# qingpingmo/OCN

Measured on AMD Instinct MI355X. Metric: candidate-edges/sec (CN predictor fwd), ogbl-collab shape, higher is better.
Workload: dtype f32

## Files before the change

### include/ocn_hip.h

```cpp
#ifndef OCN_HIP_H
#define OCN_HIP_H

#include <stdint.h>

#ifdef __cplusplus
extern "C" {
#endif

#define OCN_ABI_VERSION 9
#define OCN_EINVAL (-1)
#define OCN_ECAP   (-2)

#define OCN_ST_CAP  1
#define OCN_ST_SCAN 2
#define OCN_SCAN_POISON (-1)

#define OCN_F_CN1 1u
#define OCN_F_CN2 2u

int ocn_abi_version(void);

int64_t ocn_scan_workspace_bytes(int64_t n);

int ocn_zero_regions(void* const* ptrs, const int64_t* bytes, int32_t n, void* stream);
// ... 135 lines not shown
int64_t ocn_two_hop_window_cols(void);
int ocn_two_hop_diff_count(const int64_t* rowptrA, const int32_t* colA, const int64_t* rowptrM, const int32_t* colM,
                           int64_t n_cols, const int64_t* rows, int64_t Q, int32_t drop_self,
                           int64_t window_cols , int32_t* count , void* stream);
int ocn_two_hop_diff_fill(const int64_t* rowptrA, const int32_t* colA, const int64_t* rowptrM, const int32_t* colM,
                          int64_t n_cols, const int64_t* rows, int64_t Q, int32_t drop_self,
                          int64_t window_cols , const int64_t* off ,
                          int64_t* edges , void* stream);
int64_t ocn_two_hop_sums_window_cols(void);
int ocn_two_hop_sums_fill(const int64_t* rowptrA, const int32_t* colA, const int64_t* rowptrM, const int32_t* colM,
                          int64_t n_cols, const int64_t* rows, int64_t Q, int32_t drop_self,
                          int64_t window_cols ,
                          const float* w ,
                          int32_t wcol , const int64_t* off ,
                          int64_t* edges , float* val , void* stream);
int64_t ocn_frontier_window_cols(void);
int ocn_frontier_count(const int64_t* rowptrA, const int32_t* colA, const int64_t* rowptrM, const int32_t* colM, int64_t n_cols,
                       const int64_t* rows, int64_t Q, int32_t drop_self, int64_t window_cols ,
                       const int64_t* ptrF , const int64_t* nodeF ,
                       const int64_t* ptrS , const int64_t* nodeS ,
                       int32_t* count , void* stream);
int ocn_frontier_sums_fill(const int64_t* rowptrA, const int32_t* colA, const int64_t* rowptrM, const int32_t* colM,
                           int64_t n_cols, const int64_t* rows, int64_t Q, int32_t drop_self,
                           int64_t window_cols , const int64_t* ptrF ,
                           const int64_t* nodeF , const float* valF ,
                           const int64_t* ptrS , const int64_t* nodeS ,
                           const float* valS , const int64_t* off ,
                           int64_t* edges , float* val , void* stream);
int32_t ocn_segment_topk_max_k(void);
int ocn_segment_topk(const float* scores, const int64_t* ptr, int64_t Q, int32_t k, float* top_val, int64_t* top_pos,
                     void* stream);
int ocn_segment_rank(const float* scores, const int64_t* ptr, const int64_t* edges , int64_t Q,
                     const int64_t* tptr , const int64_t* tnode , int64_t P,
                     int64_t* rank , int64_t* pos , void* stream);

int ocn_philox4x32(const uint32_t* ctr , uint32_t key0, uint32_t key1, int64_t n, uint32_t* out ,
                   void* stream);
int ocn_complement_count(const int64_t* rowptrK, const int32_t* colK, int64_t n_cols, int32_t* count ,
                         void* stream);
int32_t ocn_sample_stage_cols(void);
int ocn_sample_complement_rows(const int64_t* rowptrK, const int32_t* colK, int64_t n_cols, const int64_t* rows, int64_t Q,
                               int64_t per, int64_t q0, uint64_t seed, int64_t* out , void* stream);
int ocn_sample_complement_pairs(const int64_t* rowptrK, const int32_t* colK, int64_t n_cols,
                                const int64_t* cptr , int64_t T, int64_t t0, uint64_t seed,
                                int64_t* out , void* stream);

int64_t ocn_sample_two_hop_window_cols(void);
int ocn_sample_two_hop(const int64_t* rowptrA, const int32_t* colA, const int64_t* rowptrM, const int32_t* colM, int64_t n_cols,
                       const int64_t* rows, int64_t Q, int32_t drop_self, int64_t window_cols ,
                       const int64_t* sptr , const int64_t* sid , int64_t q0, uint64_t seed,
                       int32_t* count , int64_t* out , void* stream);

int ocn_gather_schedule(const int32_t* gcost, int64_t n_groups, int64_t segment, int32_t* perm, void* stream);

int ocn_cn_weights_cn6(uint64_t* histA, uint64_t* histB, int64_t N, const float* innerprod, int32_t* scalars,
                       float* nip_out, const float* s2_exact , const float* s3_exact ,
                       void* stream);
int ocn_cn_gather3(const int64_t* rowptrA, const int32_t* colA, const int64_t* src, const int64_t* dst,
                   const int64_t* order, int64_t B, const int64_t* off, const uint8_t* flagsA,
                   const uint8_t* flagsB, const float* weightsA, const float* weightsB, const float* nip,
                   const float* h, int32_t H, float* xcn1, float* xcn2, float* xcn3, float* xij, void* stream);

int ocn_cn3_flags(const int64_t* rowptrA, const int32_t* colA, const int64_t* rowptrT, const int32_t* colT,
                  const uint32_t* bitmapP, int64_t bm_stride_words, const int64_t* src, const int64_t* dst,
                  const int64_t* order , int64_t B, int64_t n_cols, const int64_t* off, uint8_t* flags,
                  int64_t flags_cap, uint64_t* hist , int32_t* cnt3, int32_t* status,
                  const int64_t* nds , const int64_t* chunk_off , void* stream);

int ocn_cn_gather3_backward(const int64_t* rowptrA, const int32_t* colA, const int64_t* src, const int64_t* dst,
                            const int64_t* order, int64_t B, const int64_t* off, const uint8_t* flagsA,
                            const uint8_t* flagsB, const float* weightsA, const float* weightsB, const float* nip,
                            const float* h, int32_t H, const float* g1, const float* g2, const float* g3,
                            const float* g4, float* dh, void* stream);

int ocn_cn_gather_backward(const int64_t* rowptrA, const int32_t* colA,
                           const int64_t* src, const int64_t* dst, const int64_t* order, int64_t B,
                           const int64_t* off, const uint8_t* flags, const int32_t* wc,
                           const float* weights, const float* h, int32_t H,
                           const float* g1, const float* g2, const float* g3, float* dh, void* stream);

int64_t ocn_cn_gather_backward_det_workspace_bytes(int64_t N, int64_t B, int64_t flags_cap);
int ocn_cn_gather_backward_det(const int64_t* rowptrA, const int32_t* colA, const int64_t* src, const int64_t* dst,
                               int64_t B, const int64_t* off, const uint8_t* flags, const int32_t* wc, int64_t flags_cap,
                               const float* weights, const float* h, int64_t N, int32_t H, const float* g1,
                               const float* g2, const float* g3, float* dh, void* workspace, void* stream);
int64_t ocn_cn_gather_backward_det_keys_offset(int64_t N);
int ocn_cn_gather_backward_det_lists(const int64_t* rowptrA, const int32_t* colA, const int64_t* src, const int64_t* dst,
                                     int64_t B, const int64_t* off, const uint8_t* flags, int64_t flags_cap, int64_t N,
                                     void* workspace, void* stream);

int ocn_spmm_csr(const int64_t* rowptr, const int32_t* col, const float* val, int64_t n_rows,
                 const float* x, int32_t F, const float* pre, const float* post,
                 int32_t mode, int32_t edge_scale, int32_t self_mode,
                 float* y, void* stream);

int ocn_spmm_csr_rows(const int64_t* rowptr, const int32_t* col, const float* val, int64_t n_rows,
                      const float* x, int32_t F, const float* pre, const float* post,
                      int32_t mode, int32_t edge_scale, int32_t self_mode,
                      const int64_t* rows, int64_t n_list, float* y, void* stream);

int ocn_spmm_csr_max_arg(const int64_t* rowptr, const int32_t* col, const float* val, int64_t n_rows,
                         const float* x, int32_t F, float* y, int32_t* arg, void* stream);
int ocn_spmm_max_backward(const int64_t* rowptrT, const int32_t* colT, const float* valT, int64_t n_rows,
                          const int32_t* arg, const float* g, int32_t F, float* gx, void* stream);

int ocn_sddmm_csr(const int64_t* rowptr, const int32_t* col, const float* val , int64_t n_rows,
// ... 143 lines not shown
```

### ocn_amd/_lib.py

```python
from __future__ import annotations

import ctypes
import glob
import os
import subprocess
from ctypes import c_float, c_int32, c_int64, c_void_p

_HERE = os.path.dirname(os.path.abspath(__file__))
_ROOT = os.path.dirname(_HERE)
LIB_PATH = os.environ.get("OCN_LIB_PATH", os.path.join(_HERE, "libocn_hip.so"))
CSRC = os.path.join(_HERE, "csrc")
INCLUDE = os.path.join(_ROOT, "include")

_P = c_void_p
ABI_VERSION = 9
SIGNATURES = {
    "ocn_abi_version": (c_int32, []),
    "ocn_scan_workspace_bytes": (c_int64, [c_int64]),
    "ocn_zero_regions": (c_int32, [_P, _P, c_int32, _P]),
    "ocn_check_edges": (c_int32, [_P, _P, c_int64, c_int64, c_int64, _P, _P]),
    "ocn_edge_offsets": (c_int32, [_P, _P, c_int64, _P, _P, _P]),
    "ocn_class_order": (c_int32, [_P, _P, _P, c_int64, _P, _P, _P, _P, _P, _P]),
    "ocn_scan_i32": (c_int32, [_P, c_int64, _P, _P, _P]),
    "ocn_order_workspace_bytes": (c_int64, [c_int64]),
# ... 4 lines not shown
    "ocn_cn_flags": (c_int32, [_P, _P, _P, _P, _P, _P, _P, c_int64, _P, c_int64, _P, _P, _P, c_int64, c_int64, _P, _P, c_int64, _P,
                               _P, _P, _P, _P, _P, _P]),
    "ocn_cn_flags_rec": (c_int32, [_P, _P, _P, _P, _P, _P, _P, c_int64, _P, c_int64, _P, _P, _P, c_int64, c_int64, _P, _P, c_int64, _P,
                                   _P, _P, _P, _P, _P, _P]),
    "ocn_chunk_offsets": (c_int32, [_P, _P, _P, _P, c_int64, _P, _P, _P]),
    "ocn_walk_chunk": (c_int32, []),
    "ocn_cn_walk_flags": (c_int32, [_P, _P, _P, _P, _P, _P, c_int64, _P, _P, _P, c_int64, _P, _P, c_int64, _P, _P, _P,
                                    _P, _P]),
    "ocn_neighbor_degree_sum": (c_int32, [_P, _P, c_int64, _P, _P]),
    "ocn_walk_prep_max_batch": (c_int32, []),
    "ocn_cn_flags_small_graph_cols": (c_int32, []),
    "ocn_cn_flags_pair_min_batch": (c_int64, [c_int64]),
    "ocn_walk_prep": (c_int32, [_P, _P, _P, _P, c_int64, c_int32, _P, _P, _P, _P, _P, _P, _P, _P, _P, _P, _P, _P, _P]),
    "ocn_cn_walk_group": (c_int32, [_P, _P, _P, _P, _P, c_int64, _P, _P, _P, _P, _P, _P, _P, c_int64, _P, _P, _P, _P]),
    "ocn_walk_rev_offsets": (c_int32, [_P, _P, _P, _P, _P, c_int64, _P, _P, _P]),
    "ocn_cn_weights_cn5": (c_int32, [_P, c_int64, _P, _P, c_int32, _P, _P]),
    "ocn_cn5_column_stats": (c_int32, [_P, c_int64, _P, _P]),
    "ocn_cn_colsum_workspace_bytes": (c_int64, [c_int64, c_int64]),
    "ocn_cn_colsum_exact": (c_int32, [_P, _P, _P, c_int64, _P, _P, _P, _P, c_int64, _P, c_int64, _P, _P, _P, _P, _P, _P, _P]),
    "ocn_cn_weights_cn7": (c_int32, [_P, c_int64, c_float, _P, _P, _P]),
    "ocn_cn_gather": (c_int32, [_P, _P, _P, _P, _P, c_int64, _P, _P, _P, _P, _P, c_int32, c_int64, _P, _P, _P, _P, _P,
                                _P, _P, _P, _P, _P]),
    "ocn_cn8_pool": (c_int32, [_P, _P, _P, _P, _P, _P, _P, c_int64, _P, c_int64, _P, _P, _P, c_int64, c_int64, _P, c_int32, _P, _P,
                               _P, _P, _P, _P]),
    "ocn_cn_pool_frozen": (c_int32, [_P, _P, _P, _P, _P, _P, _P, c_int64, _P, c_int64, _P, _P, _P, c_int64, c_int64, _P, _P, c_int32, _P,
                                     _P, _P, _P, _P, _P]),
    "ocn_cn_attribution": (c_int32, [_P, _P, _P, _P, c_int64, _P, _P, _P, c_int64, _P, _P, c_int32, _P, _P, _P, _P, _P]),
    "ocn_cn_node_sums": (c_int32, [_P, _P, _P, _P, _P, _P, _P, c_int64, _P, c_int64, _P, _P, _P, c_int64, c_int64, _P, _P, _P, _P, _P,
                                   _P, _P]),
    "ocn_row_diff_stage_cols": (c_int32, []),
    "ocn_row_diff_count": (c_int32, [_P, _P, _P, _P, _P, c_int64, c_int32, _P, _P]),
    "ocn_row_diff_fill": (c_int32, [_P, _P, _P, _P, _P, c_int64, c_int32, _P, _P, _P]),
    "ocn_two_hop_window_cols": (c_int64, []),
    "ocn_two_hop_diff_count": (c_int32, [_P, _P, _P, _P, c_int64, _P, c_int64, c_int32, c_int64, _P, _P]),
    "ocn_two_hop_diff_fill": (c_int32, [_P, _P, _P, _P, c_int64, _P, c_int64, c_int32, c_int64, _P, _P, _P]),
    "ocn_two_hop_sums_window_cols": (c_int64, []),
    "ocn_two_hop_sums_fill": (c_int32, [_P, _P, _P, _P, c_int64, _P, c_int64, c_int32, c_int64, _P, c_int32, _P, _P, _P, _P]),
    "ocn_frontier_window_cols": (c_int64, []),
    "ocn_frontier_count": (c_int32, [_P, _P, _P, _P, c_int64, _P, c_int64, c_int32, c_int64, _P, _P, _P, _P, _P, _P]),
    "ocn_frontier_sums_fill": (c_int32, [_P, _P, _P, _P, c_int64, _P, c_int64, c_int32, c_int64, _P, _P, _P, _P, _P, _P, _P, _P, _P,
                                         _P]),
    "ocn_segment_topk_max_k": (c_int32, []),
    "ocn_segment_topk": (c_int32, [_P, _P, c_int64, c_int32, _P, _P, _P]),
    "ocn_segment_rank": (c_int32, [_P, _P, _P, c_int64, _P, _P, c_int64, _P, _P, _P]),
    "ocn_philox4x32": (c_int32, [_P, ctypes.c_uint32, ctypes.c_uint32, c_int64, _P, _P]),
    "ocn_complement_count": (c_int32, [_P, _P, c_int64, _P, _P]),
    "ocn_sample_stage_cols": (c_int32, []),
    "ocn_sample_complement_rows": (c_int32, [_P, _P, c_int64, _P, c_int64, c_int64, c_int64, ctypes.c_uint64, _P, _P]),
    "ocn_sample_complement_pairs": (c_int32, [_P, _P, c_int64, _P, c_int64, c_int64, ctypes.c_uint64, _P, _P]),
    "ocn_sample_two_hop_window_cols": (c_int64, []),
    "ocn_sample_two_hop": (c_int32, [_P, _P, _P, _P, c_int64, _P, c_int64, c_int32, c_int64, _P, _P, c_int64, ctypes.c_uint64, _P, _P,
                                     _P]),
    "ocn_gather_schedule": (c_int32, [_P, c_int64, c_int64, _P, _P]),
    "ocn_coo_to_csr_workspace_bytes": (c_int64, [c_int64, c_int64, c_int32, c_int32]),
    "ocn_coo_to_csr": (c_int32, [_P, _P, c_int64, c_int64, c_int64, c_int32, c_int32, _P, _P, _P, _P, _P]),
    "ocn_wgrad_workspace_bytes": (c_int64, [c_int64, c_int32, c_int32]),
    "ocn_wgrad": (c_int32, [_P, c_int64, _P, c_int64, c_int64, c_int32, c_int32, _P, _P, _P, _P]),
    "ocn_cn_weights_cn6": (c_int32, [_P, _P, c_int64, _P, _P, _P, _P, _P, _P]),
    "ocn_cn_gather3": (c_int32, [_P, _P, _P, _P, _P, c_int64, _P, _P, _P, _P, _P, _P, _P, c_int32, _P, _P, _P, _P, _P]),
    "ocn_cn3_flags": (c_int32, [_P, _P, _P, _P, _P, c_int64, _P, _P, _P, c_int64, c_int64, _P, _P, c_int64, _P, _P, _P, _P, _P, _P]),
    "ocn_cn_gather3_backward": (c_int32, [_P, _P, _P, _P, _P, c_int64, _P, _P, _P, _P, _P, _P, _P, c_int32, _P, _P, _P, _P, _P, _P]),
    "ocn_cn_gather_backward": (c_int32, [_P, _P, _P, _P, _P, c_int64, _P, _P, _P, _P, _P, c_int32, _P, _P, _P, _P, _P]),
    "ocn_cn_gather_backward_det_workspace_bytes": (c_int64, [c_int64, c_int64, c_int64]),
    "ocn_cn_gather_backward_det": (c_int32, [_P, _P, _P, _P, c_int64, _P, _P, _P, c_int64, _P, _P, c_int64, c_int32, _P, _P, _P, _P,
                                             _P, _P]),
    "ocn_cn_gather_backward_det_keys_offset": (c_int64, [c_int64]),
    "ocn_cn_gather_backward_det_lists": (c_int32, [_P, _P, _P, _P, c_int64, _P, _P, c_int64, c_int64, _P, _P]),
    "ocn_ln_drop_relu_workspace_bytes": (c_int64, [c_int32]),
    "ocn_ln_drop_relu_forward": (c_int32, [_P, _P, _P, c_float, c_float, ctypes.c_uint64, c_int32, c_int64, c_int32, _P, _P, _P]),
    "ocn_ln_drop_relu_backward": (c_int32, [_P, _P, _P, _P, _P, c_float, ctypes.c_uint64, c_int32, c_int64, c_int32, _P, _P, _P, _P, _P]),
    "ocn_dropout_keep_mask": (c_int32, [ctypes.c_uint64, c_float, c_int64, _P, _P]),
    "ocn_mix3_workspace_bytes": (c_int64, []),
    "ocn_mix3_backward": (c_int32, [_P, _P, _P, _P, _P, c_int64, _P, _P, _P, _P, _P, _P]),
    "ocn_spmm_csr": (c_int32, [_P, _P, _P, c_int64, _P, c_int32, _P, _P, c_int32, c_int32, c_int32, _P, _P]),
    "ocn_spmm_csr_rows": (c_int32, [_P, _P, _P, c_int64, _P, c_int32, _P, _P, c_int32, c_int32, c_int32, _P, c_int64, _P, _P]),
    "ocn_spmm_csr_max_arg": (c_int32, [_P, _P, _P, c_int64, _P, c_int32, _P, _P, _P]),
    "ocn_spmm_max_backward": (c_int32, [_P, _P, _P, c_int64, _P, _P, c_int32, _P, _P]),
    "ocn_sddmm_csr": (c_int32, [_P, _P, _P, c_int64, _P, _P, c_int32, _P, _P, c_int32, c_int32, c_int32, _P, _P]),
    "ocn_deg_rsqrt": (c_int32, [_P, _P, c_int64, c_float, _P, _P]),
    "ocn_spgemm_max_cols": (c_int64, []),
    "ocn_spgemm_pattern_count": (c_int32, [_P, _P, c_int64, _P, _P, c_int64, _P, _P, c_int64, _P]),
    "ocn_spgemm_pattern_fill": (c_int32, [_P, _P, c_int64, _P, _P, c_int64, _P, _P, _P]),
    "ocn_spgemm_bit_rows": (c_int32, [_P, _P, c_int64, _P, _P, c_int64, _P, c_int64, _P, _P, c_int64, _P]),
    "ocn_dense_from_csr": (c_int32, [_P, _P, c_int64, c_int64, _P, _P, _P]),
    "ocn_dense_block_mm_bits": (c_int32, [_P, _P, c_int64, c_int64, c_int32, c_int32, c_int32, c_int32, c_int32, _P, c_int64, _P]),
    "ocn_bitrows_from_csr": (c_int32, [_P, _P, c_int64, _P, c_int64, _P]),
    "ocn_bitrows_count": (c_int32, [_P, c_int64, c_int64, c_int64, _P, _P]),
    "ocn_bitrows_fill": (c_int32, [_P, c_int64, c_int64, c_int64, _P, _P, _P]),
    "ocn_csr_union_count": (c_int32, [_P, _P, _P, _P, c_int64, _P, _P]),
    "ocn_csr_union_fill": (c_int32, [_P, _P, _P, _P, c_int64, _P, _P, _P]),
    "ocn_bitrows_insert_workspace_bytes": (c_int64, [c_int64]),
    "ocn_bitrows_insert": (c_int32, [_P, _P, _P, _P, _P, _P, c_int64, c_int64, _P, c_int64, _P, _P, _P]),
    "ocn_csr_minus_count": (c_int32, [_P, _P, _P, _P, c_int64, _P, _P]),
    "ocn_csr_minus_fill": (c_int32, [_P, _P, _P, _P, c_int64, _P, _P, _P]),
    "ocn_bitrows_remove_workspace_bytes": (c_int64, [c_int64]),
    "ocn_bitrows_remove": (c_int32, [_P, _P, _P, _P, _P, _P, _P, _P, _P, _P, c_int64, c_int64, _P, c_int64, _P, _P, _P]),
    "ocn_rows_neighbourhood_workspace_bytes": (c_int64, [c_int64]),
    "ocn_rows_neighbourhood": (c_int32, [_P, _P, c_int64, _P, c_int64, _P, _P, _P]),
    "ocn_bitlist_count": (c_int32, [_P, c_int64, _P, _P]),
    "ocn_bitlist_fill": (c_int32, [_P, c_int64, _P, _P, _P]),
    "ocn_rows_ln_relu": (c_int32, [_P, _P, _P, c_float, c_int32, c_int64, c_int32, _P, _P]),
    "ocn_fill_rows": (c_int32, [_P, c_int64, c_int32, _P, _P, c_int64, _P]),
    "ocn_combine3": (c_int32, [_P, _P, _P, _P, c_int64, _P, _P]),
    "ocn_linear_panel_bytes": (c_int64, [c_int32, c_int32]),
    "ocn_linear_split_weight": (c_int32, [_P, c_int32, c_int32, _P, _P]),
    "ocn_linear_bf16x6": (c_int32, [_P, c_int64, c_int32, _P, c_int32, _P, _P, _P, c_float, c_int32, _P, _P,
# ... 114 lines not shown
```

### ocn_amd/csrc/cn_pool.hip

```cpp
#include "common.h"


constexpr int GATHER_UNR = 4;
template <int LPE, int NV, int UNR = (LPE >= 64 ? 2 * GATHER_UNR : GATHER_UNR)>
__device__ __forceinline__ void pool_range(i64 p_begin, i64 p_end, i64 a0, i64 base, int gl, int gbase,
                                           const int32_t* __restrict__ colA, const uint8_t* __restrict__ flags,
                                           const int32_t* __restrict__ wc, const float4* __restrict__ weights,
                                           const float4* __restrict__ h4, i64 rowq, float4 (&acc1)[NV],
                                           float4 (&acc2)[NV], bool full2 = false) {
  constexpr int PT = (OCN_WAVE / LPE) < 8 ? (OCN_WAVE / LPE) : 8;
  f32x2 acc[NV][4];
#pragma unroll
  for (int v = 0; v < NV; ++v) {
    acc[v][0] = f32x2{acc1[v].x, acc2[v].x}; acc[v][1] = f32x2{acc1[v].y, acc2[v].y};
    acc[v][2] = f32x2{acc1[v].z, acc2[v].z}; acc[v][3] = f32x2{acc1[v].w, acc2[v].w};
  }
  for (i64 p0 = p_begin; p0 < p_end; p0 += LPE * PT) {
    int32_t k[PT];
    unsigned f[PT];
    int32_t cv[PT];
#pragma unroll
    for (int t = 0; t < PT; ++t) {
      const i64 p = p0 + t * LPE + gl;
      k[t] = 0; f[t] = 0; cv[t] = 1;
      if (p < p_end) {
        k[t] = colA[a0 + p]; f[t] = flags[base + p];
        if (wc) cv[t] = wc[base + p];
      }
      if (full2) f[t] &= ~OCN_F_CN2;
    }
    float wa[PT], wb[PT];
#pragma unroll
    for (int t = 0; t < PT; ++t) {
      wa[t] = wb[t] = 0.f;
      if (f[t]) entry_weights(f[t], weights[k[t]], (float)cv[t], wa[t], wb[t]);
    }
#pragma unroll
    for (int t = 0; t < PT; ++t) {
      const bool need = (wa[t] != 0.f) | (wb[t] != 0.f);
      unsigned long long m = __ballot(need);
      if (LPE < 64) m = (m >> gbase) & ((1ull << (LPE & 63)) - 1ull);
      while (m) {
        int bsel[UNR];
#pragma unroll
        for (int u = 0; u < UNR; ++u) {
          bsel[u] = m ? (__ffsll((long long)m) - 1) : -1;
          m &= m - 1;
        }
        int32_t kk[UNR];
        float wwa[UNR], wwb[UNR];
        float4 x[UNR][NV];
#pragma unroll
        for (int u = 0; u < UNR; ++u) {
          const int sl = gbase + (bsel[u] < 0 ? 0 : bsel[u]);
          kk[u] = __shfl(k[t], sl, OCN_WAVE);
          wwa[u] = __shfl(wa[t], sl, OCN_WAVE);
          wwb[u] = __shfl(wb[t], sl, OCN_WAVE);
          if (bsel[u] >= 0) {
            const float4* row = h4 + (i64)kk[u] * rowq + gl;
#pragma unroll
            for (int v = 0; v < NV; ++v) x[u][v] = row[v * LPE];
          }
        }
#pragma unroll
        for (int u = 0; u < UNR; ++u) {
          if (bsel[u] >= 0) {
            const f32x2 w = {wwa[u], wwb[u]};
#pragma unroll
            for (int v = 0; v < NV; ++v) {
              axpy_pair(acc[v][0], w, x[u][v].x);
              axpy_pair(acc[v][1], w, x[u][v].y);
              axpy_pair(acc[v][2], w, x[u][v].z);
              axpy_pair(acc[v][3], w, x[u][v].w);
            }
          }
        }
      }
    }
  }
#pragma unroll
  for (int v = 0; v < NV; ++v) {
    acc1[v] = make_float4(acc[v][0].x, acc[v][1].x, acc[v][2].x, acc[v][3].x);
    acc2[v] = make_float4(acc[v][0].y, acc[v][1].y, acc[v][2].y, acc[v][3].y);
  }
}

template <int LPE, int NV>
__device__ __forceinline__ void pool_store(i64 e, i64 i, i64 j, int gl, const float4* __restrict__ h4, i64 rowq,
                                           const float4 (&acc1)[NV], const float4 (&acc2)[NV],
                                           float* __restrict__ xcn1, float* __restrict__ xcn2,
                                           float* __restrict__ xij, bool st1 = true, bool st2 = true) {
  const float4* hi = h4 + i * rowq + gl;
  const float4* hj = h4 + j * rowq + gl;
  float4* o1 = reinterpret_cast<float4*>(xcn1) + e * rowq + gl;
  float4* o2 = reinterpret_cast<float4*>(xcn2) + e * rowq + gl;
  float4* o3 = reinterpret_cast<float4*>(xij) + e * rowq + gl;
#pragma unroll
  for (int v = 0; v < NV; ++v) {
    const float4 a = hi[v * LPE], b = hj[v * LPE];
    if (st1) o1[v * LPE] = acc1[v];
    if (st2) o2[v * LPE] = acc2[v];
    o3[v * LPE] = make_float4(__fmul_rn(a.x, b.x), __fmul_rn(a.y, b.y), __fmul_rn(a.z, b.z),
                              __fmul_rn(a.w, b.w));
  }
}

#define LONG_ROW 1024

template <int LPE, int NV>
__global__ __launch_bounds__(OCN_BLOCK) void cn_gather_kernel(
    const i64* __restrict__ rowptrA, const int32_t* __restrict__ colA,
    const i64* __restrict__ src, const i64* __restrict__ dst, const i64* __restrict__ order, i64 B,
    const i64* __restrict__ off, const uint8_t* __restrict__ flags, const int32_t* __restrict__ wc,
    const float4* __restrict__ weights, const float* __restrict__ h, int H,
    float* __restrict__ xcn1, float* __restrict__ xcn2, float* __restrict__ xij,
    const i64* __restrict__ out_row,
    const int32_t* __restrict__ cnt1, const int32_t* __restrict__ cnt2,
    const u64* __restrict__ rec,
    const int32_t* __restrict__ perm,
    const float* __restrict__ rowsum) {
  constexpr int GPW = OCN_WAVE / LPE;
  const int lane = threadIdx.x & 63;
  const int gl = lane % LPE;
  const int gbase = lane - gl;
  i64 bid = blockIdx.x;
  if ((gridDim.x & 7) == 0) {
    bid = (bid & 7) * (gridDim.x >> 3) + (bid >> 3);
    if (perm) bid = perm[bid];
  }
  const i64 slot = (bid * OCN_WPB + (threadIdx.x >> 6)) * GPW + lane / LPE;
  if (slot >= B) return;
  i64 e, i, j, a0, da, base;
  bool has1, has2, full2;
  if (rec) {
    const ulonglong2* rp = reinterpret_cast<const ulonglong2*>(rec + 4 * slot);
    const ulonglong2 ra = rp[0], rb = rp[1];
    e = (i64)ra.x; i = (i64)(ra.y & 0xffffffffull); j = (i64)(ra.y >> 32);
    a0 = (i64)(rb.x & ((1ull << REC_LEN_SHIFT) - 1)); da = (i64)(rb.x >> REC_LEN_SHIFT);
    base = (i64)(rb.y & ((1ull << REC_FULL2_BIT) - 1)); has1 = (rb.y >> 62) & 1ull; has2 = rb.y >> 63;
    full2 = rowsum && ((rb.y >> REC_FULL2_BIT) & 1ull);
  } else {
    e = order ? order[slot] : slot;
    i = src[e]; j = dst[e];
    a0 = rowptrA[i]; da = rowptrA[i + 1] - a0;
    base = off[e];
    has1 = !cnt1 || cnt1[e] > 0; has2 = !cnt2 || cnt2[e] > 0;
    full2 = rowsum && cnt2 && da > 0 && (i64)cnt2[e] == da;
  }
  if (da > LONG_ROW && !full2) return;
  const float4* h4 = reinterpret_cast<const float4*>(h);
  const i64 rowq = H >> 2;
  float4 acc1[NV], acc2[NV];
#pragma unroll
  for (int v = 0; v < NV; ++v) acc1[v] = acc2[v] = make_float4(0.f, 0.f, 0.f, 0.f);
  if (has1 | (has2 & !full2)) pool_range<LPE, NV>(0, da, a0, base, gl, gbase, colA, flags, wc, weights, h4, rowq, acc1, acc2, full2);
  if (full2) {
    const float4* rs = reinterpret_cast<const float4*>(rowsum) + i * rowq + gl;
#pragma unroll
    for (int v = 0; v < NV; ++v) acc2[v] = rs[v * LPE];
  }
  pool_store<LPE, NV>(out_row ? out_row[e] : e, i, j, gl, h4, rowq, acc1, acc2, xcn1, xcn2, xij,
                      !out_row || has1, !out_row || has1 || has2);
}

template <int FPL, int HF>
__device__ __forceinline__ void chain_rows(const float2* __restrict__ w, const float* __restrict__ xs, int nr,
                                           float (&acc1)[FPL], float (&acc2)[FPL]) {
  constexpr int BLK = FPL >= 4 ? 2 : 8 / FPL;
  f32x2 acc[FPL];
#pragma unroll
  for (int q = 0; q < FPL; ++q) acc[q] = f32x2{acc1[q], acc2[q]};
  auto load = [&](int r, float2 (&w8)[BLK], float (&x8)[BLK][FPL]) {
#pragma unroll
    for (int u = 0; u < BLK; ++u) {
      w8[u] = w[r + u];
#pragma unroll
      for (int q = 0; q < FPL; ++q) x8[u][q] = xs[(r + u) * HF + q];
    }
  };
  auto add = [&](const float2 (&w8)[BLK], const float (&x8)[BLK][FPL]) {
#pragma unroll
    for (int u = 0; u < BLK; ++u)
#pragma unroll
      for (int q = 0; q < FPL; ++q) axpy_pair_lds(acc[q], f32x2{w8[u].x, w8[u].y}, x8[u][q]);
  };
  const int nb = nr / BLK;
  if (nb > 0) {
    float2 wa[BLK], wb[BLK];
    float xa[BLK][FPL], xb[BLK][FPL];
    load(0, wa, xa);
    int b = 0;
    for (; b + 2 <= nb; b += 2) {
      load((b + 1) * BLK, wb, xb);
      add(wa, xa);
      if (b + 2 < nb) load((b + 2) * BLK, wa, xa);
      add(wb, xb);
    }
    if (b < nb) add(wa, xa);
  }
  for (int r = nb * BLK; r < nr; ++r) {
    const float2 wr = w[r];
#pragma unroll
    for (int q = 0; q < FPL; ++q) axpy_pair_lds(acc[q], f32x2{wr.x, wr.y}, xs[r * HF + q]);
  }
#pragma unroll
  for (int q = 0; q < FPL; ++q) { acc1[q] = acc[q].x; acc2[q] = acc[q].y; }
}

template <int LPE, int NV, bool LONG>
constexpr int gather_wave_wpb() { return LONG ? 1 : ((size_t)OCN_WPB * OCN_WAVE * (LPE * NV * 16 + 24) > 65536 ? 2 : OCN_WPB); }

template <int LPE, int NV, bool LONG = false, int WPB = gather_wave_wpb<LPE, NV, LONG>()>
__global__ __launch_bounds__(WPB * OCN_WAVE) void cn_gather_wave_kernel(
    const i64* __restrict__ rowptrA, const int32_t* __restrict__ colA,
    const i64* __restrict__ src, const i64* __restrict__ dst, const i64* __restrict__ order, i64 B,
// ... 301 lines not shown
  pool_store<LPE, NV>(e, i, j, gl, h4, rowq, acc1, acc2, xcn1, xcn2, xij);
  float4* o3 = reinterpret_cast<float4*>(xcn3) + e * rowq + gl;
#pragma unroll
  for (int v = 0; v < NV; ++v) o3[v * LPE] = acc3[v];
}

__global__ __launch_bounds__(OCN_BLOCK) void cn_gather_generic(
    const i64* __restrict__ rowptrA, const int32_t* __restrict__ colA,
    const i64* __restrict__ src, const i64* __restrict__ dst, const i64* __restrict__ order, i64 B,
    const i64* __restrict__ off, const uint8_t* __restrict__ flags, const int32_t* __restrict__ wc,
    const float4* __restrict__ weights, const float* __restrict__ h, int H,
    float* __restrict__ xcn1, float* __restrict__ xcn2, float* __restrict__ xij,
    const i64* __restrict__ out_row) {
  const int lane = threadIdx.x & 63;
  const i64 slot = (i64)blockIdx.x * OCN_WPB + (threadIdx.x >> 6);
  if (slot >= B) return;
  const i64 e = order ? order[slot] : slot;
  const i64 i = src[e], j = dst[e];
  const i64 a0 = rowptrA[i], da = rowptrA[i + 1] - a0;
  const i64 base = off[e];
  for (int f0 = 0; f0 < H; f0 += OCN_WAVE) {
    const int ft = f0 + lane;
    const bool fin = ft < H;
    float acc1 = 0.f, acc2 = 0.f;
    for (i64 p0 = 0; p0 < da; p0 += OCN_WAVE) {
      const i64 p = p0 + lane;
      int32_t k = 0;
      unsigned f = 0;
      if (p < da) { k = colA[a0 + p]; f = flags[base + p]; }
      float wa = 0.f, wb = 0.f;
      if (f) entry_weights(f, weights[k], wc ? (float)wc[base + p] : 1.0f, wa, wb);
      unsigned long long m = __ballot((wa != 0.f) | (wb != 0.f));
      while (m) {
        const int b = __ffsll((long long)m) - 1;
        m &= m - 1;
        const int32_t kk = __shfl(k, b, OCN_WAVE);
        const float a = __shfl(wa, b, OCN_WAVE), bb = __shfl(wb, b, OCN_WAVE);
        if (fin) {
          const float x = h[(i64)kk * H + ft];
          acc1 = __fadd_rn(acc1, __fmul_rn(a, x));
          acc2 = __fadd_rn(acc2, __fmul_rn(bb, x));
        }
      }
    }
    if (fin) {
      const i64 oe = out_row ? out_row[e] : e;
      xcn1[oe * H + ft] = acc1;
      xcn2[oe * H + ft] = acc2;
      xij[oe * H + ft] = __fmul_rn(h[i * H + ft], h[j * H + ft]);
    }
  }
}

template <int LPE, int NV>
static void launch_gather(const int64_t* rowptrA, const int32_t* colA, const int64_t* src, const int64_t* dst,
                          const int64_t* order, int64_t B, const int64_t* off, const uint8_t* flags,
                          const int32_t* wc, const float* weights, const float* h, int32_t H, int64_t max_row_len,
                          float* xcn1, float* xcn2, float* xij, const int64_t* out_row, const int32_t* cnt1,
                          const int32_t* cnt2, const uint64_t* rec, const int32_t* perm, const float* rowsum, hipStream_t st) {
  const i64 epb = (i64)OCN_WPB * (OCN_WAVE / LPE);
  const bool sched = perm && rec && epb == SCHED_GROUP && ((B + epb - 1) / epb) % 8 == 0;
  bool packed = true;
  if constexpr (LPE <= 16) {
    if (B * LPE < 262144) {
      constexpr int WW = gather_wave_wpb<LPE, NV, false>();
      hipLaunchKernelGGL((cn_gather_wave_kernel<LPE, NV>), dim3((unsigned)((B + WW - 1) / WW)),
                         dim3(WW * OCN_WAVE), 0, st, (const i64*)rowptrA, colA, (const i64*)src, (const i64*)dst,
                         (const i64*)order, (i64)B, (const i64*)off, flags, wc, (const float4*)weights, h, (int)H,
                         xcn1, xcn2, xij, (const i64*)out_row, cnt2, rowsum);
      packed = false;
    }
  }
#define PACKED_ARGS (const i64*)rowptrA, colA, (const i64*)src, (const i64*)dst, (const i64*)order, (i64)B, \
                    (const i64*)off, flags, wc, (const float4*)weights, h, (int)H, xcn1, xcn2, xij,           \
                    (const i64*)out_row, cnt1, cnt2, (const u64*)rec
  if (packed)
    hipLaunchKernelGGL((cn_gather_kernel<LPE, NV>), dim3((unsigned)((B + epb - 1) / epb)), dim3(OCN_BLOCK), 0, st,
                       PACKED_ARGS, sched ? perm : (const int32_t*)nullptr, rowsum);
#undef PACKED_ARGS
#define LONG_ARGS (const i64*)rowptrA, colA, (const i64*)src, (const i64*)dst, (i64)B, (const i64*)off, flags, wc, \
                  (const float4*)weights, h, (int)H, xcn1, xcn2, xij, (const i64*)out_row, cnt2, rowsum
  if (max_row_len > LONG_ROW) {
    bool small = false;
    if constexpr (NV == 1) {
      if (B <= 4096) {
        static bool raised_dev[64] = {};
        int devid = 0;
        if (hipGetDevice(&devid) == hipSuccess && devid >= 0 && devid < 64 && !raised_dev[devid]) {
          if (hipFuncSetAttribute((const void*)cn_gather_long_kernel<LPE, NV, LONG_SMALL_THREADS>, hipFuncAttributeMaxDynamicSharedMemorySize,
                                  2 * LONG_SLAB_BYTES(LONG_SMALL_THREADS)) == hipSuccess) raised_dev[devid] = true;
        }
        hipLaunchKernelGGL((cn_gather_long_kernel<LPE, NV, LONG_SMALL_THREADS>), dim3((unsigned)B), dim3(LONG_SMALL_THREADS), 2 * LONG_SLAB_BYTES(LONG_SMALL_THREADS), st, LONG_ARGS);
        small = true;
      }
    }
    if (!small) {
      bool by_wave = false;
      if constexpr (LPE <= 16) {
        hipLaunchKernelGGL((cn_gather_wave_kernel<LPE, NV, true>), dim3((unsigned)B), dim3(OCN_WAVE), 0, st, (const i64*)rowptrA, colA, (const i64*)src, (const i64*)dst,
                           (const i64*)order, (i64)B, (const i64*)off, flags, wc, (const float4*)weights, h, (int)H,
                           xcn1, xcn2, xij, (const i64*)out_row, cnt2, rowsum);
        by_wave = true;
      }
      if (!by_wave) hipLaunchKernelGGL((cn_gather_long_kernel<LPE, NV, 256>), dim3((unsigned)B), dim3(256), 2 * LONG_SLAB_BYTES(256), st, LONG_ARGS);
    }
  }
#undef LONG_ARGS
}

extern "C" {

#define GATHER_ARGS (const i64*)rowptrA, colA, (const i64*)src, (const i64*)dst, (const i64*)order, (i64)B, (const i64*)off, \
                    flags, wc, (const float4*)weights, h, (int)H, xcn1, xcn2, xij, (const i64*)out_row
#define LAUNCH_GATHER(LPE, NV)                                                                      \
  launch_gather<LPE, NV>(rowptrA, colA, src, dst, order, B, off, flags, wc, weights, h, H, max_row_len, xcn1, xcn2, xij, out_row, cnt1, cnt2, rec, perm, rowsum, st)

int ocn_cn_gather(const int64_t* rowptrA, const int32_t* colA, const int64_t* src,
                  const int64_t* dst, const int64_t* order, int64_t B, const int64_t* off, const uint8_t* flags,
                  const int32_t* wc, const float* weights, const float* h, int32_t H,
                  int64_t max_row_len, float* xcn1, float* xcn2, float* xij, const int64_t* out_row,
                  const int32_t* cnt1, const int32_t* cnt2, const uint64_t* rec, const int32_t* perm, const float* rowsum,
                  void* stream) {
  if (B < 0 || H <= 0) return OCN_EINVAL;
  if (B == 0) return 0;
  if (!rowptrA || !src || !dst || !off || !weights || !h || !xcn1 || !xcn2 || !xij) return OCN_EINVAL;
  if (rowsum && (wc || !cnt2)) return OCN_EINVAL;
  hipStream_t st = (hipStream_t)stream;
  switch (H) {
    case 16:  LAUNCH_GATHER(4, 1); break;
    case 32:  LAUNCH_GATHER(8, 1); break;
    case 64:  LAUNCH_GATHER(16, 1); break;
    case 128: LAUNCH_GATHER(32, 1); break;
    case 256: LAUNCH_GATHER(POOL_LPE, (64 / POOL_LPE)); break;
    case 512: LAUNCH_GATHER(64, 2); break;
    default:
      hipLaunchKernelGGL(cn_gather_generic, dim3((unsigned)((B + OCN_WPB - 1) / OCN_WPB)),
                         dim3(OCN_BLOCK), 0, st, GATHER_ARGS);
  }
  return launch_status();
}

#define LAUNCH_GATHER3(LPE, NV)                                                                      \
  hipLaunchKernelGGL((cn_gather3_kernel<LPE, NV>),                                                   \
                     dim3((unsigned)((B + (i64)OCN_WPB * (OCN_WAVE / (LPE)) - 1) / ((i64)OCN_WPB * (OCN_WAVE / (LPE))))), \
                     dim3(OCN_BLOCK), 0, (hipStream_t)stream, (const i64*)rowptrA, colA, (const i64*)src,      \
                     (const i64*)dst, (const i64*)order, (i64)B, (const i64*)off, flagsA, flagsB,             \
                     (const float4*)weightsA, (const float4*)weightsB, nip, h, (int)H, xcn1, xcn2, xcn3, xij)

int ocn_cn_gather3(const int64_t* rowptrA, const int32_t* colA, const int64_t* src, const int64_t* dst,
                   const int64_t* order, int64_t B, const int64_t* off, const uint8_t* flagsA,
                   const uint8_t* flagsB, const float* weightsA, const float* weightsB, const float* nip,
                   const float* h, int32_t H, float* xcn1, float* xcn2, float* xcn3, float* xij, void* stream) {
  if (B < 0 || H <= 0) return OCN_EINVAL;
  if (B == 0) return 0;
  if (!rowptrA || !src || !dst || !off || !weightsA || !weightsB || !nip || !h || !xcn1 || !xcn2 || !xcn3 || !xij)
    return OCN_EINVAL;
  OCN_SWITCH_WIDTH(H, LAUNCH_GATHER3)
  return launch_status();
}

}
```

### ocn_amd/ops.py

```python
from __future__ import annotations

import ctypes
import os
from typing import Optional, Tuple

import torch
from torch import Tensor

from . import _lib
from ._lib import check, ptr, stream_ptr

FLAGS_NOSYNC_LIMIT = 1 << 30
validate_indices = True
stage_timer = None
LN_WIDTHS = (16, 32, 64, 128, 256, 512)
a1_bitmap_max_bytes = int(os.environ.get("OCN_A1_BITMAP_MAX_BYTES", 64 << 20))
a2_bitmap_max_bytes = 16 << 30
skip_zero_rows = True
skip_zero_min_share = 0.15
skip_zero_backoff = 32
skip_zero_min_batch = 4096
walk_two_sided = True
walk_share_min = 2
sort_edges_min_batch = 4096
# ... 1604 lines not shown
fast_linear = True
_panels: dict = {}


@_on_device
def linear_panel(weight: Tensor) -> Tensor:
    import weakref
    key = id(weight)
    hit = _panels.get(key)
    if (hit is not None and hit[0]() is weight and hit[1] == weight.data_ptr() and hit[2] == weight._version
            and hit[3] == tuple(weight.shape)):
        return hit[4]
    w = _req(weight.detach(), torch.float32, "weight", 2)
    N, K = w.shape
    panel = torch.empty(int(_lib.lib().ocn_linear_panel_bytes(N, K)), dtype=torch.uint8, device=w.device)
    check(_lib.lib().ocn_linear_split_weight(ptr(w), N, K, ptr(panel), stream_ptr()), "ocn_linear_split_weight")
    if len(_panels) > 512:
        for k in [k for k, v in _panels.items() if v[0]() is None]:
            del _panels[k]
    _panels[key] = (weakref.ref(weight), weight.data_ptr(), weight._version, (N, K), panel)
    return panel


@_on_device
def heads_panel(weight: Tensor):
    import math
    w = _req(weight.detach(), torch.float32, "weight", 2)
    N, K = w.shape
    m = float(w.abs().max().item()) if w.numel() else 0.0
    if not math.isfinite(m):
        raise ValueError("heads_panel: non-finite weight")
    sw = 13 - math.frexp(m)[1] + 1 if m > 0.0 else 0
    sw = max(-100, min(100, sw))
    panel = torch.empty(int(_lib.lib().ocn_heads_panel_bytes(N, K)), dtype=torch.uint8, device=w.device)
    check(_lib.lib().ocn_heads_split_weight(ptr(w), N, K, float(2.0 ** sw), ptr(panel), stream_ptr()), "ocn_heads_split_weight")
    return panel, float(2.0 ** -sw)


HEADS_WIDTHS = (128, 256)
train_linear = True
train_tails = os.environ.get("OCN_TRAIN_TAILS", "1") != "0"
fused_heads = True
fused_heads_min_width = 128


def heads_small_batch(max_rows: int = -1) -> int:
    return int(_lib.lib().ocn_heads_small_batch(int(max_rows)))


def flags_pair_min_batch(min_rows: int = -1) -> int:
    return int(_lib.lib().ocn_cn_flags_pair_min_batch(int(min_rows)))


@_on_device
def heads_fused(x1: Tensor, x2: Tensor, xij: Tensor, pack: dict, ranges: Optional[Tensor], y_row_map: Optional[Tensor],
                b_on_union: bool, scratch: Tensor, dump: Optional[Tensor] = None) -> Optional[Tensor]:
    for t, nm in ((x1, "xcn1"), (x2, "xcn2"), (xij, "xij")):
        _req(t, torch.float32, nm, 2)
    B, H = xij.shape
    if x1.shape != (B, H) or x2.shape != (B, H) or H not in HEADS_WIDTHS:
        raise ValueError("heads_fused: shape mismatch")
    a = _lib.OcnHeadsArgs()
    a.x[0], a.x[1], a.x[2] = x1.data_ptr(), x2.data_ptr(), xij.data_ptr()
    a.ldx, a.B, a.H = H, B, H
    for i in range(3):
        a.p_first[i] = pack["first"][i].data_ptr()
        a.p_out[i] = pack["out"][i].data_ptr()
    a.p_mid[0], a.p_mid[1] = pack["mid"][0].data_ptr(), pack["mid"][1].data_ptr()
    a.vec = pack["vec"].data_ptr()
    a.ranges = 0 if ranges is None else _req(ranges, torch.int64, "ranges").data_ptr()
    a.y_row_map = 0 if y_row_map is None else _req(y_row_map, torch.int64, "y_row_map", 1).data_ptr()
    y = None
    nconst = int(_lib.lib().ocn_heads_const_bytes(H)) // 4
    if dump is None:
        y = torch.empty((B, 1), dtype=torch.float32, device=xij.device)
        a.y = y.data_ptr()
        if _req(pack["cpark"], torch.float32, "cpark", 1).numel() != nconst:
            raise ValueError("heads_fused: constants buffer of the wrong size")
        a.cpark = pack["cpark"].data_ptr()
    else:
        if B != 1 or _req(dump, torch.float32, "dump", 1).numel() != nconst:
            raise ValueError("heads_fused: constants mode takes one row and ocn_heads_const_bytes(H) bytes")
        a.dump = dump.data_ptr()
    if scratch.numel() * scratch.element_size() < int(_lib.lib().ocn_heads_scratch_bytes(H)):
        raise ValueError("heads_fused: scratch too small")
    a.scratch = scratch.data_ptr()
    a.eps, a.ln, a.b_on_union = float(pack["eps"]), int(pack["ln"]), int(bool(b_on_union))
    _mark("mlp_glue")
    check(_lib.lib().ocn_heads_fused(ctypes.byref(a), stream_ptr()), "ocn_heads_fused")
    _mark("linear", pack["flops_per_row"] * B)
    return y


def linear_ok(x: Tensor, weight: Tensor) -> bool:
    return (fast_linear and x.is_cuda and x.dim() == 2 and x.dtype == torch.float32 and x.is_contiguous()
            and weight.shape[0] in LINEAR_WIDTHS and weight.shape[1] % 16 == 0 and weight.shape[1] == x.shape[1])


@_on_device
def linear(x: Tensor, weight: Tensor, bias: Optional[Tensor] = None, ln=None, relu: bool = False,
           dot=None, y_row_map: Optional[Tensor] = None) -> Tensor:
    _req(x, torch.float32, "x", 2)
    M, K = x.shape
    N = weight.shape[0]
    if y_row_map is not None:
        if dot is None:
# ... 147 lines not shown
```

Measured before the change: 177.0 million.

## Add paired-edge gather kernel sharing neighbor loads across two edges per wave

Adds a new gather kernel, used for the width-64-lane, NV=1 case on large batches, that processes two candidate edges per wavefront. When both edges share the same source row, the neighbor column, flag, weight and feature-row loads are done once and accumulated into both outputs. The kernel also compacts live neighbors with ballots so feature rows are fetched only for nonzero weights, with unrolled variants chosen by popcount. It trades extra branching and register pressure for fewer redundant loads and better memory-level parallelism, and is gated by a tunable minimum batch size.

Result: faster. 178.9 million (median of 6 runs) (+1.0%).

```diff
diff --git a/include/ocn_hip.h b/include/ocn_hip.h
--- a/include/ocn_hip.h
+++ b/include/ocn_hip.h
@@ -211,6 +211,7 @@
                        int32_t* count , int64_t* out , void* stream);
 
 int ocn_gather_schedule(const int32_t* gcost, int64_t n_groups, int64_t segment, int32_t* perm, void* stream);
+int64_t ocn_cn_gather_pair_min_batch(int64_t min_rows);
 
 int ocn_cn_weights_cn6(uint64_t* histA, uint64_t* histB, int64_t N, const float* innerprod, int32_t* scalars,
                        float* nip_out, const float* s2_exact , const float* s3_exact ,
diff --git a/ocn_amd/_lib.py b/ocn_amd/_lib.py
--- a/ocn_amd/_lib.py
+++ b/ocn_amd/_lib.py
@@ -80,6 +80,7 @@
     "ocn_sample_two_hop": (c_int32, [_P, _P, _P, _P, c_int64, _P, c_int64, c_int32, c_int64, _P, _P, c_int64, ctypes.c_uint64, _P, _P,
                                      _P]),
     "ocn_gather_schedule": (c_int32, [_P, c_int64, c_int64, _P, _P]),
+    "ocn_cn_gather_pair_min_batch": (c_int64, [c_int64]),
     "ocn_coo_to_csr_workspace_bytes": (c_int64, [c_int64, c_int64, c_int32, c_int32]),
     "ocn_coo_to_csr": (c_int32, [_P, _P, c_int64, c_int64, c_int64, c_int32, c_int32, _P, _P, _P, _P, _P]),
     "ocn_wgrad_workspace_bytes": (c_int64, [c_int64, c_int32, c_int32]),
diff --git a/ocn_amd/csrc/cn_pool.hip b/ocn_amd/csrc/cn_pool.hip
--- a/ocn_amd/csrc/cn_pool.hip
+++ b/ocn_amd/csrc/cn_pool.hip
@@ -2,6 +2,14 @@
 
 
 constexpr int GATHER_UNR = 4;
+
+__device__ __forceinline__ void axpy_pair4(f32x2 (&a)[4], const f32x2 w, const float x0, const float x1, const float x2,
+                                           const float x3) {
+  axpy_pair(a[0], w, x0);
+  axpy_pair(a[1], w, x1);
+  axpy_pair(a[2], w, x2);
+  axpy_pair(a[3], w, x3);
+}
 template <int LPE, int NV, int UNR = (LPE >= 64 ? 2 * GATHER_UNR : GATHER_UNR)>
 __device__ __forceinline__ void pool_range(i64 p_begin, i64 p_end, i64 a0, i64 base, int gl, int gbase,
                                            const int32_t* __restrict__ colA, const uint8_t* __restrict__ flags,
@@ -67,12 +75,7 @@
           if (bsel[u] >= 0) {
             const f32x2 w = {wwa[u], wwb[u]};
 #pragma unroll
-            for (int v = 0; v < NV; ++v) {
-              axpy_pair(acc[v][0], w, x[u][v].x);
-              axpy_pair(acc[v][1], w, x[u][v].y);
-              axpy_pair(acc[v][2], w, x[u][v].z);
-              axpy_pair(acc[v][3], w, x[u][v].w);
-            }
+            for (int v = 0; v < NV; ++v) axpy_pair4(acc[v], w, x[u][v].x, x[u][v].y, x[u][v].z, x[u][v].w);
           }
         }
       }
@@ -83,6 +86,14 @@
     acc1[v] = make_float4(acc[v][0].x, acc[v][1].x, acc[v][2].x, acc[v][3].x);
     acc2[v] = make_float4(acc[v][0].y, acc[v][1].y, acc[v][2].y, acc[v][3].y);
   }
+}
+
+__device__ __forceinline__ void pool_emit(float4* __restrict__ o1, float4* __restrict__ o2, float4* __restrict__ o3,
+                                          const float4& acc1, const float4& acc2, const float4& a, const float4& b, bool st1,
+                                          bool st2) {
+  if (st1) *o1 = acc1;
+  if (st2) *o2 = acc2;
+  *o3 = make_float4(__fmul_rn(a.x, b.x), __fmul_rn(a.y, b.y), __fmul_rn(a.z, b.z), __fmul_rn(a.w, b.w));
 }
 
 template <int LPE, int NV>
@@ -98,10 +109,7 @@
 #pragma unroll
   for (int v = 0; v < NV; ++v) {
     const float4 a = hi[v * LPE], b = hj[v * LPE];
-    if (st1) o1[v * LPE] = acc1[v];
-    if (st2) o2[v * LPE] = acc2[v];
-    o3[v * LPE] = make_float4(__fmul_rn(a.x, b.x), __fmul_rn(a.y, b.y), __fmul_rn(a.z, b.z),
-                              __fmul_rn(a.w, b.w));
+    pool_emit(o1 + v * LPE, o2 + v * LPE, o3 + v * LPE, acc1[v], acc2[v], a, b, st1, st2);
   }
 }
 
@@ -161,6 +169,227 @@
   }
   pool_store<LPE, NV>(out_row ? out_row[e] : e, i, j, gl, h4, rowq, acc1, acc2, xcn1, xcn2, xij,
                       !out_row || has1, !out_row || has1 || has2);
+}
+
+__device__ __forceinline__ float lane_f32(float v, int l) {
+  return __builtin_bit_cast(float, __builtin_amdgcn_readlane(__builtin_bit_cast(int, v), l));
+}
+
+constexpr int PAIR_UNR = 4;
+template <int V> struct pair_const { static constexpr int value = V; };
+
+__device__ __forceinline__ int32_t pair_weight_index(unsigned f, int32_t k) {
+  const unsigned long long any = __ballot(f != 0);
+  const int32_t kd = __builtin_amdgcn_readlane(k, any ? __ffsll((long long)any) - 1 : 0);
+  return f ? k : kd;
+}
+__device__ __forceinline__ unsigned long long pair_live(unsigned f, const float4& cw, float& wa, float& wb) {
+  float a = 0.f, b = 0.f;
+  entry_weights(f, cw, 1.0f, a, b);
+  wa = f ? a : 0.f; wb = f ? b : 0.f;
+  return __ballot((wa != 0.f) | (wb != 0.f));
+}
+template <int W, int LIVE>
+__device__ __forceinline__ void pair_take(unsigned long long& m, int (&sel)[W]) {
+#pragma unroll
+  for (int t = 0; t < W; ++t) {
+    sel[t] = m ? (__ffsll((long long)m) - 1) : -1;
+    if (t < LIVE) __builtin_assume(sel[t] >= 0);
+    m &= m - 1;
+  }
+}
+template <int W, int LIVE>
+__device__ __forceinline__ void pair_trip_one(unsigned long long& m, int32_t k, float wa, float wb, const float4* __restrict__ h4,
+                                              int lane, f32x2 (&acc)[4]) {
+  int sel[W];
+  pair_take<W, LIVE>(m, sel);
+  float4 x[W];
+#pragma unroll
+  for (int t = 0; t < W; ++t) x[t] = h4[(i64)__builtin_amdgcn_readlane(k, sel[t] < 0 ? sel[0] : sel[t]) * OCN_WAVE + lane];
+#pragma unroll
+  for (int t = 0; t < W; ++t)
+    if (sel[t] >= 0) axpy_pair4(acc, f32x2{lane_f32(wa, sel[t]), lane_f32(wb, sel[t])}, x[t].x, x[t].y, x[t].z, x[t].w);
+}
+__device__ __forceinline__ void pair_rows_one(unsigned long long m, int32_t k, float wa, float wb, const float4* __restrict__ h4,
+                                              int lane, f32x2 (&acc)[4]) {
+  while (m) {
+    const int c = __popcll(m);
+    if (c > 4) pair_trip_one<2 * PAIR_UNR, 5>(m, k, wa, wb, h4, lane, acc);
+    else if (c == 4) pair_trip_one<4, 4>(m, k, wa, wb, h4, lane, acc);
+    else if (c == 3) pair_trip_one<3, 3>(m, k, wa, wb, h4, lane, acc);
+    else if (c == 2) pair_trip_one<2, 2>(m, k, wa, wb, h4, lane, acc);
+    else pair_trip_one<1, 1>(m, k, wa, wb, h4, lane, acc);
+  }
+}
+template <int W, int LIVE>
+__device__ __forceinline__ void pair_trip_same(unsigned long long& mu, unsigned long long m0, unsigned long long m1, int32_t k,
+                                               float wa0, float wb0, float wa1, float wb1, const float4* __restrict__ h4, int lane,
+                                               f32x2 (&acc0)[4], f32x2 (&acc1)[4]) {
+  int sel[W];
+  pair_take<W, LIVE>(mu, sel);
+  float4 x[W];
+#pragma unroll
+  for (int t = 0; t < W; ++t) x[t] = h4[(i64)__builtin_amdgcn_readlane(k, sel[t] < 0 ? sel[0] : sel[t]) * OCN_WAVE + lane];
+#pragma unroll
+  for (int t = 0; t < W; ++t)
+    if (sel[t] >= 0) {
+      if ((m0 >> sel[t]) & 1ull) axpy_pair4(acc0, f32x2{lane_f32(wa0, sel[t]), lane_f32(wb0, sel[t])}, x[t].x, x[t].y, x[t].z, x[t].w);
+      if ((m1 >> sel[t]) & 1ull) axpy_pair4(acc1, f32x2{lane_f32(wa1, sel[t]), lane_f32(wb1, sel[t])}, x[t].x, x[t].y, x[t].z, x[t].w);
+    }
+}
+template <int W0, int LIVE0, int W1, int LIVE1>
+__device__ __forceinline__ void pair_trip_two(unsigned long long& m0, unsigned long long& m1, int32_t k0, int32_t k1, float wa0,
+                                              float wb0, float wa1, float wb1, const float4* __restrict__ h4, int lane,
+                                              f32x2 (&acc0)[4], f32x2 (&acc1)[4]) {
+  int s0[W0], s1[W1];
+  pair_take<W0, LIVE0>(m0, s0);
+  pair_take<W1, LIVE1>(m1, s1);
+  float4 x0[W0], x1[W1];
+#pragma unroll
+  for (int t = 0; t < W0; ++t) x0[t] = h4[(i64)__builtin_amdgcn_readlane(k0, s0[t] < 0 ? s0[0] : s0[t]) * OCN_WAVE + lane];
+#pragma unroll
+  for (int t = 0; t < W1; ++t) x1[t] = h4[(i64)__builtin_amdgcn_readlane(k1, s1[t] < 0 ? s1[0] : s1[t]) * OCN_WAVE + lane];
+#pragma unroll
+  for (int t = 0; t < W0; ++t)
+    if (s0[t] >= 0) axpy_pair4(acc0, f32x2{lane_f32(wa0, s0[t]), lane_f32(wb0, s0[t])}, x0[t].x, x0[t].y, x0[t].z, x0[t].w);
+#pragma unroll
+  for (int t = 0; t < W1; ++t)
+    if (s1[t] >= 0) axpy_pair4(acc1, f32x2{lane_f32(wa1, s1[t]), lane_f32(wb1, s1[t])}, x1[t].x, x1[t].y, x1[t].z, x1[t].w);
+}
+template <int W0, int LIVE0>
+__device__ __forceinline__ void pair_trip_two_pick(unsigned long long& m0, unsigned long long& m1, int32_t k0, int32_t k1,
+                                                   float wa0, float wb0, float wa1, float wb1, const float4* __restrict__ h4,
+                                                   int lane, f32x2 (&acc0)[4], f32x2 (&acc1)[4]) {
+  const int c = __popcll(m1);
+  if (c > 2) pair_trip_two<W0, LIVE0, PAIR_UNR, 3>(m0, m1, k0, k1, wa0, wb0, wa1, wb1, h4, lane, acc0, acc1);
+  else if (c == 2) pair_trip_two<W0, LIVE0, 2, 2>(m0, m1, k0, k1, wa0, wb0, wa1, wb1, h4, lane, acc0, acc1);
+  else pair_trip_two<W0, LIVE0, 1, 1>(m0, m1, k0, k1, wa0, wb0, wa1, wb1, h4, lane, acc0, acc1);
+}
+
+__global__ __launch_bounds__(OCN_BLOCK) void cn_gather_pair_kernel(
+    const int32_t* __restrict__ colA, i64 B, const uint8_t* __restrict__ flags, const float4* __restrict__ weights,
+    const float* __restrict__ h, float* __restrict__ xcn1, float* __restrict__ xcn2, float* __restrict__ xij,
+    const i64* __restrict__ out_row, const u64* __restrict__ rec, const int32_t* __restrict__ perm) {
+  constexpr int NS = 2;
+  constexpr i64 rowq = OCN_WAVE;
+  const int lane = threadIdx.x & 63, w = __builtin_amdgcn_readfirstlane(threadIdx.x >> 6);
+  i64 bid = blockIdx.x;
+  if ((gridDim.x & 7) == 0) bid = (bid & 7) * (gridDim.x >> 3) + (bid >> 3);
+  i64 grp = 2 * bid + (w >> 1);
+  if (perm) grp = perm[grp];
+  const i64 slot0 = grp * SCHED_GROUP + 2 * (w & 1);
+  if (slot0 >= B) return;
+  u64 recw = 0;
+  if (lane < 4 * NS && slot0 + (lane >> 2) < B) recw = rec[4 * slot0 + lane];
+  i64 e[NS], i[NS], j[NS], a0[NS], base[NS], n[NS];
+  bool live[NS], has1[NS], has2[NS];
+#pragma unroll
+  for (int s = 0; s < NS; ++s) {
+    u64 q[4];
+#pragma unroll
+    for (int t = 0; t < 4; ++t)
+      q[t] = (u64)(unsigned)__builtin_amdgcn_readlane((int)(unsigned)recw, 4 * s + t) |
+             ((u64)(unsigned)__builtin_amdgcn_readlane((int)(unsigned)(recw >> 32), 4 * s + t) << 32);
+    const i64 da = (i64)(q[2] >> REC_LEN_SHIFT);
+    live[s] = slot0 + s < B && da <= LONG_ROW;
+    e[s] = live[s] ? (i64)q[0] : 0;
+    i[s] = live[s] ? (i64)(q[1] & 0xffffffffull) : 0; j[s] = live[s] ? (i64)(q[1] >> 32) : 0;
+    a0[s] = (i64)(q[2] & ((1ull << REC_LEN_SHIFT) - 1));
+    base[s] = (i64)(q[3] & ((1ull << REC_FULL2_BIT) - 1)); has1[s] = (q[3] >> 62) & 1ull; has2[s] = q[3] >> 63;
+    n[s] = live[s] && (has1[s] | has2[s]) ? da : 0;
+  }
+  const bool same = live[0] && live[1] && i[0] == i[1];
+  const float4* h4 = reinterpret_cast<const float4*>(h);
+  f32x2 acc[NS][4];
+#pragma unroll
+  for (int s = 0; s < NS; ++s)
+#pragma unroll
+    for (int c = 0; c < 4; ++c) acc[s][c] = f32x2{0.f, 0.f};
+  auto round_two = [&](auto one_source, const i64 p0) {
+    constexpr bool SAME = decltype(one_source)::value != 0;
+    const i64 p = p0 + lane;
+    int32_t k[NS];
+    unsigned f[NS];
+    k[0] = colA[a0[0] + (p < n[0] ? p : n[0] - 1)];
+    k[1] = k[0];
+    if (!SAME) k[1] = colA[a0[1] + (p < n[1] ? p : n[1] - 1)];
+#pragma unroll
+    for (int s = 0; s < NS; ++s) f[s] = flags[base[s] + (p < n[s] ? p : n[s] - 1)];
+#pragma unroll
+    for (int s = 0; s < NS; ++s)
+      if (p >= n[s]) f[s] = 0;
+    int32_t wi[NS] = {pair_weight_index(SAME ? (f[0] | f[1]) : f[0], k[0]), SAME ? 0 : pair_weight_index(f[1], k[1])};
+    asm volatile("" : "+v"(wi[0]), "+v"(wi[1]));
+    float4 cw[NS];
+    cw[0] = weights[wi[0]];
+    cw[1] = cw[0];
+    if (!SAME) cw[1] = weights[wi[1]];
+    float wa[NS], wb[NS];
+    unsigned long long m[NS];
+#pragma unroll
+    for (int s = 0; s < NS; ++s) m[s] = pair_live(f[s], cw[s], wa[s], wb[s]);
+#define PAIR_SAME_TRIP(W, LIVE) pair_trip_same<W, LIVE>(mu, m[0], m[1], k[0], wa[0], wb[0], wa[1], wb[1], h4, lane, acc[0], acc[1])
+#define PAIR_TWO_TRIP(W, LIVE) pair_trip_two_pick<W, LIVE>(m[0], m[1], k[0], k[1], wa[0], wb[0], wa[1], wb[1], h4, lane, acc[0], acc[1])
+    if constexpr (SAME) {
+      unsigned long long mu = m[0] | m[1];
+      while (mu) {
+        const int c = __popcll(mu);
+        if (c > 8) PAIR_SAME_TRIP(4 * PAIR_UNR, 9);
+        else if (c > 4) PAIR_SAME_TRIP(2 * PAIR_UNR, 5);
+        else if (c == 4) PAIR_SAME_TRIP(4, 4);
+        else if (c == 3) PAIR_SAME_TRIP(3, 3);
+        else if (c == 2) PAIR_SAME_TRIP(2, 2);
+        else PAIR_SAME_TRIP(1, 1);
+      }
+    } else {
+      while (m[0] && m[1]) {
+        const int c = __popcll(m[0]);
+        if (c > 4 && __popcll(m[1]) > 4)
+          pair_trip_two<2 * PAIR_UNR, 5, 2 * PAIR_UNR, 5>(m[0], m[1], k[0], k[1], wa[0], wb[0], wa[1], wb[1], h4, lane, acc[0], acc[1]);
+        else if (c > 2) PAIR_TWO_TRIP(PAIR_UNR, 3);
+        else if (c == 2) PAIR_TWO_TRIP(2, 2);
+        else PAIR_TWO_TRIP(1, 1);
+      }
+      pair_rows_one(m[0], k[0], wa[0], wb[0], h4, lane, acc[0]);
+      pair_rows_one(m[1], k[1], wa[1], wb[1], h4, lane, acc[1]);
+    }
+#undef PAIR_SAME_TRIP
+#undef PAIR_TWO_TRIP
+  };
+  auto round_one = [&](auto which, const i64 p0) {
+    constexpr int S = decltype(which)::value;
+    const i64 p = p0 + lane;
+    const int32_t k = colA[a0[S] + (p < n[S] ? p : n[S] - 1)];
+    unsigned f = flags[base[S] + (p < n[S] ? p : n[S] - 1)];
+    if (p >= n[S]) f = 0;
+    const float4 cw = weights[pair_weight_index(f, k)];
+    float wa, wb;
+    const unsigned long long m = pair_live(f, cw, wa, wb);
+    pair_rows_one(m, k, wa, wb, h4, lane, acc[S]);
+  };
+  const i64 n_max = n[0] > n[1] ? n[0] : n[1];
+  for (i64 p0 = 0; p0 < n_max; p0 += OCN_WAVE) {
+    const bool on0 = p0 < n[0], on1 = p0 < n[1];
+    if (on0 && on1) {
+      if (same) round_two(pair_const<1>{}, p0);
+      else round_two(pair_const<0>{}, p0);
+    } else if (on0) round_one(pair_const<0>{}, p0);
+    else round_one(pair_const<1>{}, p0);
+  }
+  i64 oe[NS];
+#pragma unroll
+  for (int s = 0; s < NS; ++s) oe[s] = out_row ? out_row[e[s]] : e[s];
+  float4 xi[NS], xj[NS];
+#pragma unroll
+  for (int s = 0; s < NS; ++s) { xi[s] = h4[i[s] * rowq + lane]; xj[s] = h4[j[s] * rowq + lane]; }
+#pragma unroll
+  for (int s = 0; s < NS; ++s)
+    if (live[s])
+      pool_emit(reinterpret_cast<float4*>(xcn1) + oe[s] * rowq + lane, reinterpret_cast<float4*>(xcn2) + oe[s] * rowq + lane,
+                reinterpret_cast<float4*>(xij) + oe[s] * rowq + lane,
+                make_float4(acc[s][0].x, acc[s][1].x, acc[s][2].x, acc[s][3].x),
+                make_float4(acc[s][0].y, acc[s][1].y, acc[s][2].y, acc[s][3].y), xi[s], xj[s], !out_row || has1[s],
+                !out_row || has1[s] || has2[s]);
 }
 
 template <int FPL, int HF>
@@ -568,6 +797,8 @@
   }
 }
 
+static int64_t g_gather_pair_min_batch = 32768;
+
 template <int LPE, int NV>
 static void launch_gather(const int64_t* rowptrA, const int32_t* colA, const int64_t* src, const int64_t* dst,
                           const int64_t* order, int64_t B, const int64_t* off, const uint8_t* flags,
@@ -590,6 +821,15 @@
 #define PACKED_ARGS (const i64*)rowptrA, colA, (const i64*)src, (const i64*)dst, (const i64*)order, (i64)B, \
                     (const i64*)off, flags, wc, (const float4*)weights, h, (int)H, xcn1, xcn2, xij,           \
                     (const i64*)out_row, cnt1, cnt2, (const u64*)rec
+  if constexpr (LPE == OCN_WAVE && NV == 1) {
+    const i64 n_groups = (B + epb - 1) / epb;
+    if (rec && !wc && !rowsum && B >= g_gather_pair_min_batch && (!sched || (n_groups >> 3) % 2 == 0)) {
+      hipLaunchKernelGGL(cn_gather_pair_kernel, dim3((unsigned)((n_groups + 1) / 2)), dim3(OCN_BLOCK), 0, st, colA, (i64)B, flags,
+                         (const float4*)weights, h, xcn1, xcn2, xij, (const i64*)out_row, (const u64*)rec,
+                         sched ? perm : (const int32_t*)nullptr);
+      packed = false;
+    }
+  }
   if (packed)
     hipLaunchKernelGGL((cn_gather_kernel<LPE, NV>), dim3((unsigned)((B + epb - 1) / epb)), dim3(OCN_BLOCK), 0, st,
                        PACKED_ARGS, sched ? perm : (const int32_t*)nullptr, rowsum);
@@ -656,7 +896,13 @@
   return launch_status();
 }
 
-#define LAUNCH_GATHER3(LPE, NV)                                                                      \
+int64_t ocn_cn_gather_pair_min_batch(int64_t min_rows) {
+  const int64_t prev = g_gather_pair_min_batch;
+  if (min_rows >= 0) g_gather_pair_min_batch = min_rows;
+  return prev;
+}
+
+#define LAUNCH_GATHER3(LPE, NV)                                                                     \
   hipLaunchKernelGGL((cn_gather3_kernel<LPE, NV>),                                                   \
                      dim3((unsigned)((B + (i64)OCN_WPB * (OCN_WAVE / (LPE)) - 1) / ((i64)OCN_WPB * (OCN_WAVE / (LPE))))), \
                      dim3(OCN_BLOCK), 0, (hipStream_t)stream, (const i64*)rowptrA, colA, (const i64*)src,      \
diff --git a/ocn_amd/ops.py b/ocn_amd/ops.py
--- a/ocn_amd/ops.py
+++ b/ocn_amd/ops.py
@@ -1680,6 +1680,10 @@
     return int(_lib.lib().ocn_cn_flags_pair_min_batch(int(min_rows)))
 
 
+def gather_pair_min_batch(min_rows: int = -1) -> int:
+    return int(_lib.lib().ocn_cn_gather_pair_min_batch(int(min_rows)))
+
+
 @_on_device
 def heads_fused(x1: Tensor, x2: Tensor, xij: Tensor, pack: dict, ranges: Optional[Tensor], y_row_map: Optional[Tensor],
                 b_on_union: bool, scratch: Tensor, dump: Optional[Tensor] = None) -> Optional[Tensor]:
```
